# davidsd/sdpb

Hardware: AMD Instinct MI355X
Metric: interior-point iterations/sec at --precision 512 (higher is better)
Workload: dtype mw576 (fixed-width multi-word float, 18x32-bit limbs; Q syrk: exact integer product of a fixed-point image with 509 fraction bits)

## Files before the change

sdpb_amd/csrc/kernels.hpp:

```cpp
#pragma once
#include "dev.hpp"
#include "mw_wave.hpp"
#include "tiledot.hpp"

#include <algorithm>
#include <cmath>
#include <cstdlib>

namespace sdpb
{
using mw::Mw;
using mw::Acc;
constexpr int WG = 256;

template <int NL> MW_HD Mw<NL> mat_ld(const Batch &b, const MatDesc &d, int i, int j)
{
  return mw::load<NL>(b.p, (size_t)d.off + (size_t)i + (size_t)j * (size_t)d.ld);
}
template <int NL> MW_HD void mat_st(const Batch &b, const MatDesc &d, int i, int j, const Mw<NL> &v)
{
  mw::store<NL>(b.p, (size_t)d.off + (size_t)i + (size_t)j * (size_t)d.ld, v);
}

template <int NL, int STRIDE> MW_HD Mw<NL> smem_ld(const uint32_t *s, int idx)
// ... 1794 lines not shown
#endif
}

template <int FX> constexpr bool fx_two_level()
{
#ifdef SDPB_SYRK_ONE_LEVEL
  return false;
#else
  return FX % 4 == 0 && FX <= 32;
#endif
}
template <int NL> constexpr int fx_limbs() { return (NL - 2 >= 14 && (NL - 2) % 4 != 0) ? ((NL - 2 + 3) / 4) * 4 : NL - 2; }
#ifndef SDPB_TOOM4_MAX_FX
#define SDPB_TOOM4_MAX_FX 48
#endif
template <int FX> constexpr bool fx_toom4()
{
#if defined(SDPB_SYRK_ONE_LEVEL) || defined(SDPB_SYRK_NO_TOOM4)
  return false;
#else
  return FX % 4 == 0 && FX >= 16 && FX <= SDPB_TOOM4_MAX_FX;
#endif
}
template <int FX> constexpr bool fx_toom4k()
{
#if defined(SDPB_SYRK_NO_TOOM4K)
  return false;
#else
  return fx_toom4<FX>() && (FX == 16 || FX == 24 || FX == 32);
#endif
}
template <int FX> constexpr bool fx_toom5k()
{
#if defined(SDPB_SYRK_NO_TOOM5K)
  return false;
#else
  return fx_toom4k<FX>() && FX == 16;
#endif
}
constexpr int T5_LB = 28;
constexpr uint32_t T5_MASK = (1u << T5_LB) - 1u;
constexpr int T5_H = 55;
template <int FX> constexpr int fx_nprod() { return fx_toom5k<FX>() ? 27 : 21; }
template <int FX> constexpr int fx_part_limbs() { return fx_toom5k<FX>() ? 5 : 2 * (FX / 8) + 1; }
template <int FX> constexpr int toom_wb() { return fx_toom5k<FX>() ? 102 : 32 * (FX / 4) - (fx_toom4k<FX>() ? 6 : 4); }
template <int FX> constexpr int fx_planes()
{
  return fx_toom5k<FX>() ? 27 * 2 : fx_toom4k<FX>() ? 21 * (FX / 8) : fx_toom4<FX>() ? 7 * (FX / 4) : fx_two_level<FX>() ? 9 * (FX / 4) : 3 * (FX / 2);
}
template <int FX> constexpr int fx_frac_bits()
{
  return fx_toom5k<FX>() ? 5 * toom_wb<FX>() - 1 : fx_toom4<FX>() ? 4 * toom_wb<FX>() - 1 : fx_two_level<FX>() ? 32 * FX - 7 : 32 * FX - 3;
}
template <int FX> constexpr size_t fx_image_stride(size_t rows, size_t cols, int rb)
{
  return fx_toom4k<FX>() ? (rows + rb - 1) / rb * rb * cols + 64 : rows * cols;
}
template <int FX> constexpr int syrk_tile_edge() { return fx_toom4k<FX>() ? 32 : 16; }

template <int BIT0, int NB, int W, int OUT> MW_HD void bits_slice(const uint32_t (&x)[W], uint32_t (&out)[OUT])
{
  constexpr int q = BIT0 / 32, r = BIT0 % 32;
#pragma unroll
  for(int i = 0; i < OUT; ++i)
    {
      const uint32_t lo = (q + i < W) ? x[q + i < W ? q + i : 0] : 0u;
      const uint32_t hi = (q + i + 1 < W) ? x[q + i + 1 < W ? q + i + 1 : 0] : 0u;
      uint32_t v = r ? ((lo >> r) | (hi << ((32 - r) & 31))) : lo;
      const int left = NB - 32 * i;
      if(left <= 0)
        v = 0;
      else if(left < 32)
        v &= (1u << (left & 31)) - 1u;
      out[i] = v;
    }
}

template <int W, int A> MW_HD void add_shifted(uint32_t (&w)[W], const uint32_t (&x)[A], int sh, bool negate)
{
  const int q = sh >> 5, r = sh & 31;
  uint64_t cy = negate ? 1u : 0u;
  const uint32_t mask = negate ? 0xffffffffu : 0u;
#pragma unroll
  for(int k = 0; k < W; ++k)
    {
      const int i0 = k - q;
      uint32_t lo = 0, hi = 0;
#pragma unroll
      for(int t = 0; t < A; ++t)
        {
          lo = (t == i0 - 1) ? x[t] : lo;
          hi = (t == i0) ? x[t] : hi;
        }
      const uint32_t limb = r ? ((hi << r) | (lo >> (32 - r))) : hi;
      const uint64_t s = (uint64_t)w[k] + (uint64_t)(limb ^ mask) + cy;
      w[k] = (uint32_t)s;
      cy = s >> 32;
    }
}

template <int FX> MW_HD void fx_store2(const uint32_t (&mag)[FX], bool negative, uint32_t *fx, size_t fx_stride, size_t idx);
template <int FX> MW_HD void fx_store4(const uint32_t (&mag)[FX], bool negative, uint32_t *fx, size_t fx_stride, size_t idx);
template <int FX> MW_HD void fx_store5(const uint32_t (&mag)[FX], bool negative, uint32_t *fx, size_t fx_stride, size_t idx);
template <int FX> MW_HD void fx_store(const uint32_t (&mag)[FX], bool negative, uint32_t *fx, size_t fx_stride, size_t idx)
{
  constexpr int M = FX / 2;
  static_assert(FX % 2 == 0 && FX >= 4, "FX = NL - 2 is even");
  if constexpr(fx_toom5k<FX>())
    {
// ... 534 lines not shown
    z_sub<Z>(t, w[1]);
#pragma unroll
    for(int k = 0; k < Z; ++k)
      w[1][k] = t[k];
  }
  z_addmul<Z>(w[5], w[3], 8, true);
  z_divexact<Z>(w[5], 9, 0x38E38E39u);
  z_sub<Z>(w[3], w[5]);
  z_divexact<Z>(w[1], 15, 0xEEEEEEEFu);
  z_add<Z>(w[1], w[5]);
  z_sar<Z>(w[1], 1);
  z_sub<Z>(w[5], w[1]);
}

template <int NL, int FX>
__global__ void __launch_bounds__(WG) k_normalize_fx(mw::CPtr PT, size_t count, int N, mw::CPtr inv_norm, uint32_t *fx, size_t fx_stride)
{
  constexpr int FB = fx_frac_bits<FX>();
  for(size_t idx = (size_t)blockIdx.x * WG + threadIdx.x; idx < count; idx += (size_t)gridDim.x * WG)
    {
      const Mw<NL> t = mw::mul(mw::load<NL>(PT, idx), mw::load<NL>(inv_norm, idx % N));
      uint32_t w[NL];
      bool sat = false;
      if(mw::is_zero(t))
        {
#pragma unroll
          for(int i = 0; i < NL; ++i)
            w[i] = 0;
        }
      else
        {
#pragma unroll
          for(int i = 0; i < NL; ++i)
            w[i] = t.m[i];
          const int s = 32 * NL - FB - t.e;
          if(t.e >= 1)
            sat = true;
          else if(s >= 32 * NL)
            {
#pragma unroll
              for(int i = 0; i < NL; ++i)
                w[i] = 0;
            }
          else
            {
              mw::shr_limbs<NL>(w, (uint32_t)s >> 5);
              mw::shr_bits<NL>(w, (uint32_t)s & 31u);
            }
        }
      uint32_t v[FX];
#pragma unroll
      for(int i = 0; i < FX; ++i)
        v[i] = sat ? ((i == FX - 1) ? ((1u << (FB % 32)) - 1u) : 0xffffffffu) : w[i];
      fx_store<FX>(v, t.neg != 0, fx, fx_stride, idx);
    }
}

template <int FX> __global__ void __launch_bounds__(WG) k_fx_from_int(const uint32_t *in, size_t in_stride, size_t count, uint32_t *fx, size_t fx_stride)
{
  const size_t idx = (size_t)blockIdx.x * WG + threadIdx.x;
  if(idx >= count)
    return;
  uint32_t v[FX];
#pragma unroll
  for(int i = 0; i < FX; ++i)
    v[i] = in[(size_t)(i + 1) * in_stride + idx];
  fx_store<FX>(v, in[idx] != 0, fx, fx_stride, idx);
}

template <int FX>
__global__ void __launch_bounds__(WG) k_fx_colsum(const uint32_t *fx, size_t fx_stride, unsigned nrows, int N, unsigned rows_per_slice, uint32_t *partial)
{
  constexpr int M = FX / 2, A = M + 2;
  const int col = blockIdx.x * 64 + (threadIdx.x & 63), phase = threadIdx.x >> 6;
  const unsigned r_begin = blockIdx.y * rows_per_slice, r_end = (r_begin + rows_per_slice < nrows) ? r_begin + rows_per_slice : nrows;
  uint32_t sl[A], sh[A];
#pragma unroll
  for(int k = 0; k < A; ++k)
    sl[k] = sh[k] = 0;
  if(col < N)
    for(unsigned r = r_begin + phase; r < r_end; r += 4)
      {
        const size_t e = (size_t)r * N + col;
        uint64_t cl = 0, ch = 0;
#pragma unroll
        for(int k = 0; k < A; ++k)
          {
            const uint64_t l = (uint64_t)sl[k] + (k < M ? fx[(size_t)(k < M ? k : 0) * fx_stride + e] : 0u) + cl;
            const uint64_t h = (uint64_t)sh[k] + (k < M ? fx[(size_t)(M + (k < M ? k : 0)) * fx_stride + e] : 0u) + ch;
            sl[k] = (uint32_t)l;
            cl = l >> 32;
            sh[k] = (uint32_t)h;
            ch = h >> 32;
          }
      }
  __shared__ uint32_t sm[3 * 2 * A * 64];
  if(phase > 0)
    {
#pragma unroll
      for(int k = 0; k < A; ++k)
        {
          sm[((phase - 1) * 2 * A + k) * 64 + (threadIdx.x & 63)] = sl[k];
          sm[((phase - 1) * 2 * A + A + k) * 64 + (threadIdx.x & 63)] = sh[k];
        }
    }
  __syncthreads();
  if(phase == 0 && col < N)
    {
      for(int p = 0; p < 3; ++p)
        {
          uint64_t cl = 0, ch = 0;
#pragma unroll
          for(int k = 0; k < A; ++k)
            {
              const uint64_t l = (uint64_t)sl[k] + sm[(p * 2 * A + k) * 64 + threadIdx.x] + cl;
              const uint64_t h = (uint64_t)sh[k] + sm[(p * 2 * A + A + k) * 64 + threadIdx.x] + ch;
              sl[k] = (uint32_t)l;
              cl = l >> 32;
              sh[k] = (uint32_t)h;
              ch = h >> 32;
// ... 803 lines not shown
    }
  if constexpr(TOOM)
    {
      if(i < N && j <= i)
        {
          const size_t o = (size_t)tile * 256 + threadIdx.x;
#pragma unroll
          for(int g = 0; g < NG; ++g)
            if(g < ngs)
              {
#pragma unroll
                for(int k = 0; k < A2; ++k)
                  acc[(size_t)((sweep * NG + g) * A2 + k) * acc_stride + o] = g2[g][k];
              }
        }
    }
  else if constexpr(SWEEPS == 3)
    second_level(sweep, 0);
  }
  if constexpr(TOOM)
    return;
  else
  {
  if constexpr(SWEEPS == 1)
    {
#pragma unroll
      for(int k = 0; k < 3; ++k)
        second_level(k, 3 * k);
    }
  if(i < N && j <= i)
    {
      sub_limbs<A>(x[2], x[0]);
      sub_limbs<A>(x[2], x[1]);
      uint32_t w[W];
#pragma unroll
      for(int k = 0; k < W; ++k)
        w[k] = k < A ? x[0][k < A ? k : 0] : 0u;
      add_shifted<W, A>(w, x[2], 32 * M - 3, false);
      add_shifted<W, A>(w, x[1], 64 * M - 6, false);
      const size_t o = packed ? (size_t)tile * 256 + threadIdx.x : (size_t)i + (size_t)j * N;
#pragma unroll
      for(int k = 0; k < W; ++k)
        acc[(size_t)k * acc_stride + o] = w[k];
    }
  }
}

#ifndef SDPB_SYRK3_PREFETCH
#define SDPB_SYRK3_PREFETCH 1
#endif
#ifndef SDPB_SYRK3_WAVES
#define SDPB_SYRK3_WAVES 3
#endif
#ifndef SDPB_SYRK3_NBUF
#define SDPB_SYRK3_NBUF 2
#endif
template <int FX, int RBG>
__global__ void __launch_bounds__(WG, SDPB_SYRK3_WAVES)
  k_syrk_fx3(const uint32_t *__restrict__ fx_in, size_t fx_stride, unsigned nrows, int N, uint32_t *acc, size_t acc_stride,
             const uint32_t *tile_list, int ntile, int nsplit, unsigned rows_per_split, int gsplit, int order)
{
  constexpr bool LAZY = fx_toom5k<FX>();
  constexpr int M3 = FX / 8, A3 = fx_part_limbs<FX>(), NPROD = fx_nprod<FX>();
  static_assert(M3 >= 2 && M3 <= 4 && (!LAZY || (M3 == 2 && RBG <= 32)), "accumulators of 2 x 2 outputs in registers; 2 x 32 rows between carries");
  constexpr int ROWW = 32 * M3, UPR = ROWW / 4, NPAIR = RBG * UPR, GL = NPAIR / WG;
  static_assert(NPAIR % WG == 0, "a pass stages a whole number of units per lane");
  const uint32_t *fx = (const uint32_t *)__builtin_assume_aligned(fx_in, 4);
  const int nitem = ntile * nsplit * gsplit, per = (nitem + 7) / 8;
  int item = (int)(blockIdx.x % 8) * per + (int)(blockIdx.x / 8);
  if(order == 1)
    {
      const int tper = (ntile + 7) / 8, slot = (int)(blockIdx.x / 8), sgx = slot / tper, tl = (int)(blockIdx.x % 8) * tper + slot % tper;
      if(sgx >= nsplit * gsplit || tl >= ntile)
        return;
      item = sgx * ntile + tl;
    }
  else if((int)(blockIdx.x / 8) >= per || item >= nitem)
    return;
  const int sg = item / ntile, tile = item % ntile, split = sg / gsplit;
  const int prod_begin = (sg % gsplit) * (NPROD / gsplit), prod_end = prod_begin + NPROD / gsplit;
  const unsigned row_begin = (unsigned)split * rows_per_split;
  const unsigned row_end = (row_begin + rows_per_split < nrows && split + 1 < nsplit) ? row_begin + rows_per_split : nrows;
  acc += (size_t)split * NPROD * A3 * acc_stride;
  const uint32_t tt = tile_list[tile];
  const int ti = (int)(tt >> 16), tj = (int)(tt & 0xffffu);
  const int li = threadIdx.x & 15, lj = threadIdx.x >> 4;
  const int i0 = ti * 32 + li, j0 = tj * 32 + lj;
  const bool half_i = ti * 32 + 16 < N, half_j = tj * 32 + 16 < N;
  const int mask = 1 | (half_i ? 2 : 0) | ((half_j && tj < ti) ? 4 : 0) | ((half_i && half_j) ? 8 : 0);
#if defined(__HIP_DEVICE_COMPILE__) && !defined(SDPB_SYRK2_NO_GLDS)
  constexpr int NBUF = LAZY ? SDPB_SYRK3_NBUF : 2;
#else
  constexpr int NBUF = 2;
#endif
  static_assert(NBUF == 2 || NBUF == 3, "double or triple buffering");
  __shared__ __attribute__((aligned(16))) uint32_t sa[NBUF * NPAIR * 4 + 64];
  __shared__ __attribute__((aligned(16))) uint32_t sb[NBUF * NPAIR * 4 + 64];
  uint64_t cc[4][2 * M3 - 1];
  uint32_t hh[4][2 * M3 - 1];
  uint64_t dd[4][2 * M3 - 1];
#if defined(__HIP_DEVICE_COMPILE__) && !defined(SDPB_SYRK2_NO_GLDS)
  constexpr bool DIRECT = true;
#else
  constexpr bool DIRECT = false;
#endif
  uint32_t va[DIRECT ? 1 : GL][4], vb[DIRECT ? 1 : GL][4];
  uint32_t offa[GL], offb[GL];
#pragma unroll
  for(int t = 0; t < GL; ++t)
    {
      const int e = threadIdx.x + t * WG;
      const int unit = e % UPR, rr = e / UPR;
      offa[t] = (uint32_t)(((size_t)rr * N + ti * 32) * M3 + 4 * unit);
      offb[t] = (uint32_t)(((size_t)rr * N + tj * 32) * M3 + 4 * unit);
    }
  auto fetch = [&](int g, unsigned r0, int into) __attribute__((always_inline)) {
    const uint32_t *base = fx + ((size_t)g * fx_stride + (size_t)r0 * (size_t)N) * M3;
#pragma unroll
    for(int t = 0; t < GL; ++t)
      {
        if constexpr(DIRECT)
          {
#if defined(__HIP_DEVICE_COMPILE__)
            const int wbase = (into * NPAIR + t * WG + (int)(threadIdx.x & ~63u)) * 4;
            __builtin_amdgcn_global_load_lds((const __attribute__((address_space(1))) void *)(base + offa[t]),
                                             (__attribute__((address_space(3))) void *)(sa + wbase), 16, 0, 0);
            __builtin_amdgcn_global_load_lds((const __attribute__((address_space(1))) void *)(base + offb[t]),
                                             (__attribute__((address_space(3))) void *)(sb + wbase), 16, 0, 0);
#endif
          }
        else
          {
#pragma unroll
            for(int l = 0; l < 4; ++l)
              {
                va[t][l] = base[offa[t] + l];
                vb[t][l] = base[offb[t] + l];
              }
          }
      }
  };
  auto store = [&](int buf) __attribute__((always_inline)) {
    if constexpr(!DIRECT)
      {
#pragma unroll
        for(int t = 0; t < GL; ++t)
          {
            const int e = threadIdx.x + t * WG;
            piece_store<4>(sa + (buf * NPAIR + e) * 4, va[t]);
            piece_store<4>(sb + (buf * NPAIR + e) * 4, vb[t]);
          }
      }
  };
  auto rows = [&](auto mask_c, int buf, uint64_t (&c)[4][2 * M3 - 1], uint32_t (&h)[4][2 * M3 - 1]) __attribute__((always_inline)) {
    constexpr int MASK = decltype(mask_c)::value;
#if defined(__HIP_DEVICE_COMPILE__) && !defined(SDPB_SYRK3_NO_ASM)
    constexpr bool ASM_ROWS = (M3 == 2);
#else
    constexpr bool ASM_ROWS = false;
#endif
    if constexpr(ASM_ROWS)
      {
#if defined(__HIP_DEVICE_COMPILE__)
    typedef uint32_t u32x4 __attribute__((ext_vector_type(4)));
    const uint32_t la = (uint32_t)(uintptr_t)(__attribute__((address_space(3))) uint32_t *)(sa + buf * NPAIR * 4 + li * M3);
    const uint32_t lb = (uint32_t)(uintptr_t)(__attribute__((address_space(3))) uint32_t *)(sb + buf * NPAIR * 4 + lj * M3);
#define FX3_P(C, H, X, Y) "v_mad_u64_u32 %" #C ", vcc, %" #X ", %" #Y ", %" #C "\n\tv_addc_co_u32 %" #H ", vcc, 0, %" #H ", vcc\n\t"
#define FX3_L(C, X, Y) "v_mad_u64_u32 %" #C ", vcc, %" #X ", %" #Y ", %" #C "\n\t"
#define FX3_MAC_BOTH(o0, o1, a0x, a0y, a1x, a1y, bx, by)                                                                                   \
  if constexpr(LAZY)                                                                                                                       \
    asm volatile(FX3_L(0, 6, 10) FX3_L(3, 8, 10) FX3_L(1, 6, 11) FX3_L(4, 8, 11) FX3_L(1, 7, 10) FX3_L(4, 9, 10) FX3_L(2, 7, 11)           \
                   FX3_L(5, 9, 11)                                                                                                         \
                 : "+v"(c[o0][0]), "+v"(c[o0][1]), "+v"(c[o0][2]), "+v"(c[o1][0]), "+v"(c[o1][1]), "+v"(c[o1][2])                          \
                 : "v"(a0x), "v"(a0y), "v"(a1x), "v"(a1y), "v"(bx), "v"(by)                                                                \
                 : "vcc");                                                                                                                 \
  else                                                                                                                                     \
  asm volatile(FX3_P(0, 6, 12, 16) FX3_P(3, 9, 14, 16) FX3_P(1, 7, 12, 17) FX3_P(4, 10, 14, 17) FX3_P(1, 7, 13, 16) FX3_P(4, 10, 15, 16)   \
                 FX3_P(2, 8, 13, 17) FX3_P(5, 11, 15, 17)                                                                                  \
               : "+v"(c[o0][0]), "+v"(c[o0][1]), "+v"(c[o0][2]), "+v"(c[o1][0]), "+v"(c[o1][1]), "+v"(c[o1][2]), "+v"(h[o0][0]),           \
                 "+v"(h[o0][1]), "+v"(h[o0][2]), "+v"(h[o1][0]), "+v"(h[o1][1]), "+v"(h[o1][2])                                            \
               : "v"(a0x), "v"(a0y), "v"(a1x), "v"(a1y), "v"(bx), "v"(by)                                                                  \
               : "vcc")
#define FX3_MAC_ONE(o0, ax, ay, bx, by)                                                                                                    \
  if constexpr(LAZY)                                                                                                                       \
    asm volatile(FX3_L(0, 3, 5) FX3_L(1, 3, 6) FX3_L(1, 4, 5) FX3_L(2, 4, 6)                                                               \
                 : "+v"(c[o0][0]), "+v"(c[o0][1]), "+v"(c[o0][2])                                                                          \
                 : "v"(ax), "v"(ay), "v"(bx), "v"(by)                                                                                      \
                 : "vcc");                                                                                                                 \
  else                                                                                                                                     \
  asm volatile(FX3_P(0, 3, 6, 8) FX3_P(1, 4, 6, 9) FX3_P(1, 4, 7, 8) FX3_P(2, 5, 7, 9)                                                     \
               : "+v"(c[o0][0]), "+v"(c[o0][1]), "+v"(c[o0][2]), "+v"(h[o0][0]), "+v"(h[o0][1]), "+v"(h[o0][2])                            \
               : "v"(ax), "v"(ay), "v"(bx), "v"(by)                                                                                        \
               : "vcc")
#define FX3_ROW(O0, O1)                                                                                                                    \
  {                                                                                                                                        \
    u32x4 va, vb;                    \
    asm volatile("ds_read2_b64 %0, %2 offset0:" #O0 " offset1:" #O1 "\n\tds_read2_b64 %1, %3 offset0:" #O0 " offset1:" #O1                \
                 "\n\ts_waitcnt lgkmcnt(0)"                                                                                                \
                 : "=&v"(va), "=&v"(vb)                                                                                                    \
                 : "v"(xa), "v"(xb)                                                                                                        \
                 : "memory");                                                                                                              \
    if constexpr(MASK == 15)                                                                                                               \
      {                                                                                                                                    \
        FX3_MAC_BOTH(0, 1, va.x, va.y, va.z, va.w, vb.x, vb.y);                                                                            \
        FX3_MAC_BOTH(2, 3, va.x, va.y, va.z, va.w, vb.z, vb.w);                                                                            \
      }                                                                                                                                    \
    else if constexpr(MASK == 11)                                                                                                          \
      {                                                                                                                                    \
        FX3_MAC_BOTH(0, 1, va.x, va.y, va.z, va.w, vb.x, vb.y);                                                                            \
        FX3_MAC_ONE(3, va.z, va.w, vb.z, vb.w);                                                                                            \
      }                                                                                                                                    \
    else if constexpr(MASK == 5)                                                                                                           \
      {                                                                                                                                    \
        FX3_MAC_ONE(0, va.x, va.y, vb.x, vb.y);                                                                                            \
        FX3_MAC_ONE(2, va.x, va.y, vb.z, vb.w);                                                                                            \
      }                                                                                                                                    \
    else                                                                                                                                   \
      FX3_MAC_ONE(0, va.x, va.y, vb.x, vb.y);                                                                                              \
  }
    static_assert(RBG % 4 == 0 && M3 == 2, "four rows per trip, offsets in units of 8 bytes");
#if SDPB_SYRK3_PREFETCH
#define FX3_MACS(va, vb)                                                                                                                   \
  if constexpr(MASK == 15)                                                                                                                 \
    {                                                                                                                                      \
      FX3_MAC_BOTH(0, 1, va.x, va.y, va.z, va.w, vb.x, vb.y);                                                                              \
      FX3_MAC_BOTH(2, 3, va.x, va.y, va.z, va.w, vb.z, vb.w);                                                                              \
    }                                                                                                                                      \
  else if constexpr(MASK == 11)                                                                                                            \
    {                                                                                                                                      \
      FX3_MAC_BOTH(0, 1, va.x, va.y, va.z, va.w, vb.x, vb.y);                                                                              \
      FX3_MAC_ONE(3, va.z, va.w, vb.z, vb.w);                                                                                              \
    }                                                                                                                                      \
  else if constexpr(MASK == 5)                                                                                                             \
    {                                                                                                                                      \
      FX3_MAC_ONE(0, va.x, va.y, vb.x, vb.y);                                                                                              \
      FX3_MAC_ONE(2, va.x, va.y, vb.z, vb.w);                                                                                              \
    }                                                                                                                                      \
  else                                                                                                                                     \
    FX3_MAC_ONE(0, va.x, va.y, vb.x, vb.y);
#ifdef SDPB_SYRK3_EXPERIMENT_HALF_LDS
#define FX3_NEXT(wa, wb, ra, rb, O0, O1)                                                                                                   \
  asm volatile("s_waitcnt lgkmcnt(0)\n\tds_read2_b64 %2, %4 offset0:" #O0 " offset1:" #O1                                                  \
               : "+v"(wa), "+v"(wb), "=&v"(ra), "+v"(rb)                                                                                   \
               : "v"(xa), "v"(xb)                                                                                                          \
               : "memory")
#else
#define FX3_NEXT(wa, wb, ra, rb, O0, O1)                                                                                                   \
  asm volatile("s_waitcnt lgkmcnt(0)\n\tds_read2_b64 %2, %4 offset0:" #O0 " offset1:" #O1 "\n\tds_read2_b64 %3, %5 offset0:" #O0            \
               " offset1:" #O1                                                                                                             \
               : "+v"(wa), "+v"(wb), "=&v"(ra), "=&v"(rb)                                                                                  \
               : "v"(xa), "v"(xb)                                                                                                          \
               : "memory")
#endif
    u32x4 a0, b0, a1, b1;
    {
      const uint32_t xa = la, xb = lb;
      asm volatile("ds_read2_b64 %0, %2 offset0:0 offset1:16\n\tds_read2_b64 %1, %3 offset0:0 offset1:16" : "=&v"(a0), "=&v"(b0) : "v"(xa), "v"(xb) : "memory");
    }
#pragma unroll 1
    for(int rr = 0; rr < RBG; rr += 4)
      {
        const uint32_t xa = la + rr * 256, xb = lb + rr * 256;
        FX3_NEXT(a0, b0, a1, b1, 32, 48);
        FX3_MACS(a0, b0)
        FX3_NEXT(a1, b1, a0, b0, 64, 80);
        FX3_MACS(a1, b1)
        FX3_NEXT(a0, b0, a1, b1, 96, 112);
        FX3_MACS(a0, b0)
        FX3_NEXT(a1, b1, a0, b0, 128, 144);
        FX3_MACS(a1, b1)
      }
    asm volatile("s_waitcnt lgkmcnt(0)" : "+v"(a0), "+v"(b0)::"memory");
#undef FX3_NEXT
#undef FX3_MACS
#else
#pragma unroll 1
    for(int rr = 0; rr < RBG; rr += 4)
      {
        const uint32_t xa = la + rr * 256, xb = lb + rr * 256;
        FX3_ROW(0, 16)
        FX3_ROW(32, 48)
        FX3_ROW(64, 80)
        FX3_ROW(96, 112)
      }
#endif
#undef FX3_ROW
#undef FX3_MAC_ONE
#undef FX3_MAC_BOTH
#undef FX3_P
#undef FX3_L
#endif
      }
    else
      {
        const uint32_t *pa = sa + buf * NPAIR * 4 + li * M3, *pb = sb + buf * NPAIR * 4 + lj * M3;
#pragma unroll SDPB_SYRK2_UNROLL
        for(int rr = 0; rr < RBG; ++rr)
          {
            uint32_t a0[M3], a1[M3], b0[M3], b1[M3];
            piece_load<M3>(pa + rr * ROWW, a0);
            piece_load<M3>(pb + rr * ROWW, b0);
            if constexpr((MASK & 10) != 0)
              piece_load<M3>(pa + rr * ROWW + 16 * M3, a1);
            if constexpr((MASK & 12) != 0)
              piece_load<M3>(pb + rr * ROWW + 16 * M3, b1);
            if constexpr(LAZY)
              {
                auto lazy = [&](const uint32_t (&x)[M3], const uint32_t (&y)[M3], uint64_t (&cs)[2 * M3 - 1]) {
                  cs[0] += (uint64_t)x[0] * y[0];
                  cs[1] += (uint64_t)x[0] * y[1] + (uint64_t)x[1] * y[0];
                  cs[2] += (uint64_t)x[1] * y[1];
                };
                lazy(a0, b0, c[0]);
                if constexpr((MASK & 2) != 0)
                  lazy(a1, b0, c[1]);
                if constexpr((MASK & 4) != 0)
                  lazy(a0, b1, c[2]);
                if constexpr((MASK & 8) != 0)
                  lazy(a1, b1, c[3]);
              }
            else
              {
            SyrkColumns<M3, 0>::run(a0, b0, c[0], h[0]);
            if constexpr((MASK & 2) != 0)
              SyrkColumns<M3, 0>::run(a1, b0, c[1], h[1]);
            if constexpr((MASK & 4) != 0)
              SyrkColumns<M3, 0>::run(a0, b1, c[2], h[2]);
            if constexpr((MASK & 8) != 0)
              SyrkColumns<M3, 0>::run(a1, b1, c[3], h[3]);
              }
          }
      }
  };
  for(int prod = prod_begin; prod < prod_end; ++prod)
    {
#pragma unroll
      for(int o = 0; o < 4; ++o)
#pragma unroll
        for(int k = 0; k < 2 * M3 - 1; ++k)
          {
            cc[o][k] = 0;
            hh[o][k] = 0;
          }
#pragma unroll
      for(int o = 0; o < 4; ++o)
#pragma unroll
        for(int k = 0; k < 2 * M3 - 1; ++k)
          dd[o][k] = 0;
      auto carry_columns = [&](bool all) __attribute__((always_inline)) {
        if constexpr(LAZY)
          {
#pragma unroll
            for(int o = 0; o < 4; ++o)
              {
                dd[o][1] += cc[o][1] >> 32;
                cc[o][1] &= 0xffffffffull;
              }
            if(all)
// ... 103 lines not shown
  const size_t pidx = (size_t)blockIdx.x * WG + threadIdx.x;
  const int prod = blockIdx.y;
  int i, j;
  if(pidx >= total || !syrk_packed_decode<32>(pidx, tile_list, N, col0, col1, i, j))
    return;
  uint32_t out[A3];
  uint64_t cy = 0;
#pragma unroll
  for(int k = 0; k < A3; ++k)
    {
#pragma unroll 8
      for(int s = 0; s < nsplit; ++s)
        cy += part[(((size_t)s * NPROD + prod) * A3 + k) * part_stride + pidx];
      out[k] = (uint32_t)cy;
      cy >>= 32;
    }
#pragma unroll
  for(int k = 0; k < A3; ++k)
    part[((size_t)prod * A3 + k) * part_stride + pidx] = out[k];
}

constexpr uint32_t inv_mod_2_32(uint32_t c)
{
  uint32_t x = c;
  for(int i = 0; i < 5; ++i)
    x *= 2u - c * x;
  return x;
}
constexpr int T5_Z = 10;
MW_HD void toom5_value(const uint32_t *fx, size_t fx_stride, int point, size_t e, uint32_t (&w)[4])
{
  const PiecePair lo = *reinterpret_cast<const PiecePair *>(fx + ((size_t)(3 * point + 0) * fx_stride + e) * 2);
  const PiecePair hi = *reinterpret_cast<const PiecePair *>(fx + ((size_t)(3 * point + 1) * fx_stride + e) * 2);
  w[0] = lo.w[0] | (lo.w[1] << 28);
  w[1] = (lo.w[1] >> 4) | (hi.w[0] << 23);
  w[2] = (hi.w[0] >> 9) | (hi.w[1] << 19);
  w[3] = hi.w[1] >> 13;
}
template <int FX>
__global__ void __launch_bounds__(WG) k_fx_colsum5(const uint32_t *fx, size_t fx_stride, unsigned nrows, int N, unsigned rows_per_slice, uint32_t *partial)
{
  constexpr int A = 5, G = 5;
  const int lane = threadIdx.x & 63, col = blockIdx.x * 64 + lane, phase = threadIdx.x >> 6;
  const unsigned r_begin = blockIdx.y * rows_per_slice, r_end = (r_begin + rows_per_slice < nrows) ? r_begin + rows_per_slice : nrows;
  uint32_t sum[G][A];
#pragma unroll
  for(int u = 0; u < G; ++u)
#pragma unroll
    for(int k = 0; k < A; ++k)
      sum[u][k] = 0;
  if(col < N)
    for(unsigned r = r_begin + phase; r < r_end; r += 4)
      {
        const size_t e = (size_t)r * N + col;
#pragma unroll
        for(int u = 0; u < G; ++u)
          {
            const int point = u == 0 ? 0 : u == 1 ? 1 : u == 2 ? 3 : u == 3 ? 5 : 8;
            uint32_t src[4];
            toom5_value(fx, fx_stride, point, e, src);
            uint64_t cy = 0;
#pragma unroll
            for(int k = 0; k < A; ++k)
              {
                const uint64_t t = (uint64_t)sum[u][k] + (k < 4 ? src[k < 4 ? k : 0] : 0u) + cy;
                sum[u][k] = (uint32_t)t;
                cy = t >> 32;
              }
          }
      }
  __shared__ uint32_t sm[3 * G * A * 64];
  if(phase > 0)
    {
#pragma unroll
      for(int u = 0; u < G; ++u)
#pragma unroll
        for(int k = 0; k < A; ++k)
          sm[(((phase - 1) * G + u) * A + k) * 64 + lane] = sum[u][k];
    }
  __syncthreads();
  if(phase == 0 && col < N)
    {
      for(int p = 0; p < 3; ++p)
#pragma unroll
        for(int u = 0; u < G; ++u)
          {
            uint64_t cy = 0;
#pragma unroll
            for(int k = 0; k < A; ++k)
              {
                const uint64_t t = (uint64_t)sum[u][k] + sm[((p * G + u) * A + k) * 64 + lane] + cy;
                sum[u][k] = (uint32_t)t;
                cy = t >> 32;
              }
          }
#pragma unroll
      for(int u = 0; u < G; ++u)
#pragma unroll
        for(int k = 0; k < A; ++k)
          partial[(((size_t)blockIdx.y * G + u) * A + k) * N + col] = sum[u][k];
    }
}
template <int FX>
__global__ void __launch_bounds__(WG)
  k_fx_colsum5_final(const uint32_t *partial, int nslices, int N, uint32_t *acc, size_t acc_stride, uint32_t *toomU, unsigned long long nrows_local)
{
  constexpr int A = 5, G = 5, W = 2 * FX + 2, WB = toom_wb<FX>(), Z = T5_Z;
// ... 1031 lines not shown
```

sdpb_amd/csrc/solver.hpp:

```cpp
#pragma once
#include "kernels.hpp"
#include "mw_host.hpp"

#include <algorithm>
#include <atomic>
#include <chrono>
#include <cstring>
#include <limits>
#include <map>
#include <memory>
#include <sstream>
#include <string>
#include <utility>

namespace sdpb
{
struct SolverError : std::runtime_error
{
  int code;
  SolverError(int c, const std::string &m) : std::runtime_error(m), code(c) {}
};

struct Collectives
{
// ... 1646 lines not shown
    if(budget_words && need > budget_words)
      {
        const size_t bw = std::max(budget_words, tile_words);
        int nchunk = (int)cdiv(need, bw);
        for(;; ++nchunk)
          {
            int ct = (int)cdiv(ntile, nchunk);
            if(ct >= 64)
              ct = (int)(cdiv(ct, 8) * 8);
            pl.chunk_tiles = std::min(ntile, ct);
            pl.nsplit_first = syrk_splits_for(pl.chunk_tiles, nrows, bw);
            if((size_t)pl.nsplit_first * tile_words * pl.chunk_tiles <= bw || pl.chunk_tiles <= 1)
              break;
          }
        pl.nchunk = (int)cdiv(ntile, pl.chunk_tiles);
      }
    pl.part_words = (size_t)pl.nsplit_first * tile_words * pl.chunk_tiles;
    return pl;
  }
  size_t window_budget_words() const { return max_shared_bytes_ ? std::max<size_t>(1, max_shared_bytes_ / sizeof(uint32_t)) : syrk_part_default_words_; }
  size_t syrk_part_budget_words(size_t image_words) const
  {
    if(const char *e = std::getenv("SDPB_HIP_SYRK_PART_BYTES"))
      return std::max<size_t>(1, (size_t)std::max(1.0, std::atof(e)) / sizeof(uint32_t));
    const size_t w = window_budget_words();
    return std::max<size_t>(1, w - std::min(image_words, w / 2));
  }
  size_t syrk_part_budget_words() const { return syrk_part_budget_words(fx_.n); }
  struct QWindow
  {
    unsigned chunk_rows = 0;
    int chunks = 0;
    size_t stride = 0;
    size_t image_words = 0;
    size_t budget_words = 0;
    bool bound_exceeded = false;
  };
  QWindow qwin_;
  size_t image_budget_words() const
  {
    if(const char *e = std::getenv("SDPB_HIP_SYRK_IMAGE_BYTES"))
      return std::max<size_t>(1, (size_t)std::max(1.0, std::atof(e)) / sizeof(uint32_t));
    return std::max<size_t>(1, window_budget_words() / 2);
  }
  static size_t image_words_for(size_t rows, size_t cols) { return image_stride(rows, cols) * fx_planes<FX>() + 4; }
  QWindow q_window(unsigned nrows, int N, bool one_chunk = false) const
  {
    QWindow w;
    w.budget_words = image_budget_words();
    const unsigned quantum = (unsigned)SYRK_RB;
    unsigned rows = std::max(nrows, 1u);
    if(!one_chunk && image_words_for(rows, (size_t)N) > w.budget_words)
      {
        const size_t per_row = (size_t)N * fx_planes<FX>();
        const size_t fixed = (size_t)64 * fx_planes<FX>() + 4;
        size_t fit = w.budget_words > fixed ? (w.budget_words - fixed) / per_row : 0;
        fit = fit / quantum * quantum;
        if(fit < quantum)
          {
            fit = quantum;
            w.bound_exceeded = true;
          }
        const unsigned f = (unsigned)cdiv(nrows, fit);
        unsigned cr = (unsigned)(cdiv(cdiv(nrows, f), quantum) * quantum);
        if(SYRK_SPLIT_ROWS && cr > SYRK_SPLIT_ROWS)
          {
            const unsigned up = (unsigned)(cdiv(cr, SYRK_SPLIT_ROWS) * SYRK_SPLIT_ROWS);
            if(up <= fit)
              cr = up;
          }
        rows = cr;
      }
    if(one_chunk && image_words_for(rows, (size_t)N) > w.budget_words)
      w.bound_exceeded = true;
    w.chunk_rows = rows;
    w.chunks = nrows ? (int)cdiv(nrows, rows) : 1;
    w.stride = image_stride((size_t)rows, (size_t)N);
    w.image_words = w.stride * fx_planes<FX>() + 4;
    return w;
  }
  template <class MakeImage, class Mark>
  void syrk_G_windows(const QWindow &w, unsigned nrows, int N, DevBuf<uint32_t> &fx, uint32_t *acc, size_t acc_stride, DevBuf<uint32_t> &acc2,
                      uint32_t *colsum_partial, const uint32_t *tiles_dev, DevBuf<uint32_t> &part, uint32_t *toomU, MakeImage &&make, Mark &&mark)
  {
    if(w.chunks > 1 && acc2.n < acc_stride * ACCW)
      acc2.alloc(acc_stride * ACCW);
    for(int c = 0; c < w.chunks; ++c)
      {
        const size_t r0 = (size_t)c * w.chunk_rows;
        const unsigned rows = (unsigned)std::min<size_t>(w.chunk_rows, nrows - r0);
        if(c > 0 && rows < w.chunk_rows)
          HIP_CHECK(hipMemsetAsync(fx.p, 0, fx.n * sizeof(uint32_t), stream_));
        make(r0, rows);
        uint32_t *out = c == 0 ? acc : acc2.p;
        const unsigned slices = (unsigned)std::min<size_t>(128, std::max<size_t>(1, cdiv((size_t)rows, 64)));
        syrk_column_sums(fx.p, w.stride, rows, N, out, acc_stride, colsum_partial, slices, toomU);
        if(c == 0)
          mark();
        syrk_G(fx.p, w.stride, rows, N, out, acc_stride, tiles_dev, part, toomU, -1, 0, -1, w.image_words);
        if(c > 0)
          launch(k_acc_add_tri<ACCW>, dim3(cdiv(acc_stride, WG)), dim3(WG), stream_, acc, (const uint32_t *)acc2.p, acc_stride, N);
      }
    last_windows_ = w.chunks;
  }
  int last_windows_ = 1;
  void syrk_G(const uint32_t *fx, size_t fx_stride, unsigned nrows, int N, uint32_t *acc, size_t acc_stride, const uint32_t *tiles_dev,
              DevBuf<uint32_t> &part, const uint32_t *toomU = nullptr, int ntile_sub = -1, int col0 = 0, int col1 = -1, size_t image_words = 0)
// ... 964 lines not shown
  {
    std::vector<std::pair<const char *, const char *>> tok;
    split_numbers(txt, tok);
    if((int)tok.size() != rows * cols)
      throw SolverError(4, "op_int_syrk: wrong element count");
    const size_t cnt = (size_t)rows * cols;
    std::vector<uint32_t> h(cnt * (FX + 1), 0);
    for(int c = 0; c < cols; ++c)
      for(int r = 0; r < rows; ++r)
        {
          const char *s = tok[(size_t)c * rows + r].first, *e = tok[(size_t)c * rows + r].second;
          bool negative = false;
          if(*s == '-')
            {
              negative = true;
              ++s;
            }
          mw::BigNat n;
          for(; s < e; ++s)
            {
              if(*s < '0' || *s > '9')
                throw SolverError(4, "op_int_syrk: not an integer");
              if(n.w.empty())
                {
                  if(*s != '0')
                    n.w.push_back((uint32_t)(*s - '0'));
                }
              else
                n.mul_small(10, (uint32_t)(*s - '0'));
            }
          if(n.w.size() > (size_t)FX || (n.w.size() == (size_t)FX && (n.w[FX - 1] >> (sdpb::fx_frac_bits<FX>() % 32)) != 0))
            throw SolverError(4, "op_int_syrk: |value| >= 2^" + std::to_string(sdpb::fx_frac_bits<FX>()));
          const size_t idx = (size_t)r * cols + c;
          for(size_t k = 0; k < n.w.size(); ++k)
            h[(k + 1) * cnt + idx] = n.w[k];
          h[idx] = (negative && !n.w.empty()) ? 1u : 0u;
        }
    DevBuf<uint32_t> staged, fx, acc, acc2, partial;
    staged.upload(h);
    const QWindow win = q_window((unsigned)rows, cols);
    image_alloc(fx, win.stride);
    const size_t as = (size_t)cols * cols + cols;
    acc.alloc(as * ACCW);
    const unsigned slices = (unsigned)std::min<size_t>(128, std::max<size_t>(1, cdiv((size_t)rows, 64)));
    partial.alloc((size_t)slices * COLSUM_WORDS * cols);
    DevBuf<uint32_t> tu;
    tu.alloc(TOOMU_WORDS * cols);
    DevBuf<uint32_t> tl;
    tl.upload(syrk_tile_order(cols, 0, nullptr, SYRK_EDGE));
    DevBuf<uint32_t> part;
    syrk_G_windows(win, (unsigned)rows, cols, fx, acc.p, as, acc2, partial.p, (const uint32_t *)tl.p, part, tu.p,
                   [&](size_t r0, unsigned nr) {
                     const size_t n = (size_t)nr * cols;
                     launch(k_fx_from_int<FX>, dim3(cdiv(n, WG)), dim3(WG), stream_, (const uint32_t *)staged.p + r0 * (size_t)cols, cnt, n, fx.p, win.stride);
                   },
                   [] {});
    launch(k_syrk_unbias<FX>, dim3(cdiv((size_t)cols * cols, WG)), dim3(WG), stream_, acc.p, as, cols, (unsigned long long)rows, (size_t)0,
           (size_t)cols * cols);
    HIP_CHECK(hipStreamSynchronize(stream_));
    std::vector<uint32_t> a = acc.download();
    std::string out;
    for(int j = 0; j < cols; ++j)
      for(int i = 0; i < cols; ++i)
        {
          const size_t idx = (size_t)i + (size_t)j * cols;
          if(i < j)
            {
              out += "0\n";
              continue;
            }
          mw::BigNat n;
          n.w.resize(ACCW);
          for(int k = 0; k < ACCW; ++k)
            n.w[k] = a[(size_t)k * as + idx];
          const bool negative = n.w[ACCW - 1] >> 31;
          if(negative)
            {
              uint64_t carry = 1;
              for(auto &w : n.w)
                {
                  const uint64_t s = (uint64_t)(~w) + carry;
                  w = (uint32_t)s;
                  carry = s >> 32;
                }
            }
          n.trim();
          std::string dig;
          while(!n.is_zero())
            {
              uint32_t rem = n.div_small(1000000000u);
              for(int k = 0; k < 9; ++k)
                {
                  dig.push_back((char)('0' + rem % 10));
                  rem /= 10;
                }
            }
          while(!dig.empty() && dig.back() == '0')
            dig.pop_back();
          if(dig.empty())
            dig = "0";
          else if(negative)
            dig.push_back('-');
          out.append(dig.rbegin(), dig.rend());
          out += "\n";
        }
    return out;
  }
// ... 14 lines not shown
```

sdpb_amd/workmodel.py:

```python
from __future__ import annotations

from typing import Dict, Sequence


def shapes(dims: Sequence[int], num_points: Sequence[int]):
    for m, K in zip(dims, num_points):
        P = K * m * (m + 1) // 2
        n0 = m * ((K + 1) // 2)
        n1 = m * K - n0
        yield m, K, P, (n0, n1), m * K


def macs_per_iteration(dims, num_points, N) -> Dict[str, float]:
    w = dict(cholesky_XY=0.0, pairings=0.0, schur=0.0, schur_cholesky=0.0, schur_trsm=0.0, syrk_Q=0.0,
             cholesky_Q=0.0, XY=0.0, search_direction=0.0, step_length=0.0, residues=0.0)
    for m, K, P, ns, q in shapes(dims, num_points):
        for n in ns:
            w["cholesky_XY"] += 2 * n ** 3 / 3.0
            w["pairings"] += 2.5 * n * n * q + n * q * q
            w["XY"] += n ** 3
            w["search_direction"] += 2 * 7 * n ** 3
            w["step_length"] += 2 * (2 * n ** 3 + 6 * n ** 3)
            w["residues"] += n * n * K
        w["schur"] += 8.0 * P * P
# ... 16 lines not shown
        t += 4 * q * q + P * P
        t += P * P + 2 * P * N
        t += P * N
    t += N * (N + 1) / 2 + N * N
    return t * bytes_per_number


COMPILED_LIMBS = (6, 10, 16, 18, 24, 26, 34, 42, 50, 66)
HBM_BYTES = 288 * 10 ** 9


def limbs_for(precision: int) -> int:
    want = 2 * ((precision + 127) // 64)
    for nl in COMPILED_LIMBS:
        if nl >= want:
            return nl
    raise ValueError(f"--precision {precision} is beyond the compiled widths")


def _fx(nl: int):
    fx = nl - 2
    if fx >= 14 and fx % 4:
        fx += 4 - fx % 4
    toom4 = fx >= 16 and fx % 4 == 0
    toom4k = fx in (16, 24, 32)
    toom5k = fx == 16
    two = fx % 4 == 0
    words = 54 if toom5k else 21 * (fx // 8) if toom4k else 7 * (fx // 4) if toom4 else 9 * (fx // 4) if two else 3 * (fx // 2)
    planes = 135 if toom5k else 21 * (2 * (fx // 8) + 1) if toom4k else 7 * (2 * (fx // 4) + 1) if toom4 else 2 * fx + 2
    rb = (16 if fx >= 32 else 32) if two else (16 if fx <= 24 else 8)
    waves = 3 if toom4k else (3 if fx <= 16 else 2)
    return fx, words, 32 if toom4k else 16, planes, rb, waves, toom4, toom4k


def syrk_row_splits(ntile: int, nrows: int, slots: int, rb: int, max_rows: int) -> int:
    import math
    smin = 1
    while max_rows and smin < 32 and nrows // smin > max_rows and nrows // (smin + 1) >= 64 * rb:
        smin += 1
    best, best_eff = smin, 0.0
    for s in range(smin, 33):
        if s > smin and nrows // s < 64 * rb:
            break
        items = ntile * s
        eff = items / (math.ceil(items / slots) * slots)
        if eff > best_eff + 0.02:
            best, best_eff = s, eff
    return best


def q_window(rows: int, N: int, nl: int, image_budget_bytes: int):
    fx, words, edge, planes, rb, waves, toom4, toom4k = _fx(nl)

    def image_bytes(r):
        stride = (-(-r // rb) * rb * N + 64) if toom4k else r * N
        return (max(stride, 1) * words + 4) * 4
    r = max(rows, 1)
    budget_words = max(1, image_budget_bytes // 4)
    if image_bytes(r) // 4 > budget_words:
        per_row = N * words
        fixed = 64 * words + 4
        fit = ((budget_words - fixed) // per_row if budget_words > fixed else 0) // rb * rb
        fit = max(fit, rb)
        f = -(-rows // fit)
        cr = -(-(-(-rows // f)) // rb) * rb
        if toom4k and cr > 2560:
            up = -(-cr // 2560) * 2560
            if up <= fit:
                cr = up
        r = cr
    return r, (-(-rows // r) if rows else 1), image_bytes(r)


def planned_footprint(dims, num_points, N, precision, owners=None, rank=0, world=1, num_cus=256, hbm_bytes=HBM_BYTES,
                      max_shared_bytes=0, dist_cholq=False, free_bytes=None) -> Dict[str, float]:
    nl = limbs_for(precision)
    W = 4 * (nl + 1)
    fx, words, edge, planes, rb, waves, toom4, toom4k = _fx(nl)
    psd = bases = scaled = E = pair = schur = bt = vecn = rows = jl = 0
    for j, (m, K, P, ns, q) in enumerate(shapes(dims, num_points)):
        if owners is not None and owners[j] != rank:
            continue
        jl += 1
        d = K - 1
        pr = m * (m + 1) // 2
        for n, r in zip(ns, (d // 2 + 1, (d + 1) // 2)):
            psd += n * n
            vecn += n
            bases += r * K
            scaled += K * pr * r
            E += n * q
            pair += q * q
        schur += P * P
        bt += N * P
        rows += P
    out = {"psd_state_and_scratch": 13 * max(psd, 1) * W, "bases_and_pairings": (2 * max(bases, 1) + max(scaled, 1) + 4 * max(E, 1) + 2 * max(pair, 1)) * W,
           "schur_blocks": 2 * max(schur, 1) * W, "B": max(bt, 1) * W, "P": max(bt, 1) * W}
    accw = 2 * fx + 2
    q_bytes = 2 * N * N * W + (N * N + N) * accw * 4
    if world > 1:
        q_bytes += (N * (N + 1) // 2 + N) * accw * 8
        if dist_cholq:
            pb = 16 if nl > 34 else 32
            q_bytes += ((N * pb + pb * pb + pb) * (nl + 1) + 2) * 4
    out["Q"] = q_bytes
    out["vectors_and_small"] = (5 * max(rows, 1) + 6 * max(vecn, 1) + 8 * N + 2 * max(jl, 1) * N) * W
    rest = sum(out.values())
    free = (hbm_bytes if free_bytes is None else free_bytes) - rest
    reserve = hbm_bytes // 16 + (1 << 30)
    window = max_shared_bytes or max(min(max(free - reserve, 0), hbm_bytes // 8), 64 << 20)
    chunk_rows, windows, image = q_window(rows, N, nl, max(window // 2, 4))
    out["P_fixed_point_image"] = image
    if windows > 1:
# ... 19 lines not shown
```

Measured before the change: 6.141.

## Interleave column slots in toom5k fixed-point image for 128-bit LDS reads

Changes the fixed-point image layout for the toom5k path so that columns c and c+16 within each 32-column group sit in adjacent slots, with rows padded to a multiple of 32. The lazy syrk inner loop can then fetch both operands for a row with a single ds_read_b128 instead of ds_read2_b64, and it is unrolled over 8, 16 or 32-row trips. Producers, the colsum kernel, window sizing and the Python work model are updated to the new addressing. This adds padding memory and index arithmetic on the image writers, and depends on every consumer agreeing on the permutation.

```diff
diff --git a/sdpb_amd/csrc/kernels.hpp b/sdpb_amd/csrc/kernels.hpp
--- a/sdpb_amd/csrc/kernels.hpp
+++ b/sdpb_amd/csrc/kernels.hpp
@@ -1870,9 +1870,18 @@
 {
   return fx_toom5k<FX>() ? 5 * toom_wb<FX>() - 1 : fx_toom4<FX>() ? 4 * toom_wb<FX>() - 1 : fx_two_level<FX>() ? 32 * FX - 7 : 32 * FX - 3;
 }
+template <int FX> constexpr int fx_col_slot(int c) { return fx_toom5k<FX>() ? 32 * (c / 32) + 2 * (c % 16) + (c % 32) / 16 : c; }
+template <int FX> constexpr size_t fx_row_slots(size_t cols) { return fx_toom5k<FX>() ? (cols + 31) / 32 * 32 : cols; }
+template <int FX> MW_HD size_t fx_elem(size_t idx, int N)
+{
+  if constexpr(fx_toom5k<FX>())
+    return idx / (size_t)N * fx_row_slots<FX>((size_t)N) + (size_t)fx_col_slot<FX>((int)(idx % (size_t)N));
+  else
+    return idx;
+}
 template <int FX> constexpr size_t fx_image_stride(size_t rows, size_t cols, int rb)
 {
-  return fx_toom4k<FX>() ? (rows + rb - 1) / rb * rb * cols + 64 : rows * cols;
+  return fx_toom4k<FX>() ? (rows + rb - 1) / rb * rb * fx_row_slots<FX>(cols) + 64 : rows * cols;
 }
 template <int FX> constexpr int syrk_tile_edge() { return fx_toom4k<FX>() ? 32 : 16; }
 
@@ -2513,11 +2522,12 @@
 #pragma unroll
       for(int i = 0; i < FX; ++i)
         v[i] = sat ? ((i == FX - 1) ? ((1u << (FB % 32)) - 1u) : 0xffffffffu) : w[i];
-      fx_store<FX>(v, t.neg != 0, fx, fx_stride, idx);
-    }
-}
-
-template <int FX> __global__ void __launch_bounds__(WG) k_fx_from_int(const uint32_t *in, size_t in_stride, size_t count, uint32_t *fx, size_t fx_stride)
+      fx_store<FX>(v, t.neg != 0, fx, fx_stride, fx_elem<FX>(idx, N));
+    }
+}
+
+template <int FX>
+__global__ void __launch_bounds__(WG) k_fx_from_int(const uint32_t *in, size_t in_stride, size_t count, int N, uint32_t *fx, size_t fx_stride)
 {
   const size_t idx = (size_t)blockIdx.x * WG + threadIdx.x;
   if(idx >= count)
@@ -2526,7 +2536,7 @@
 #pragma unroll
   for(int i = 0; i < FX; ++i)
     v[i] = in[(size_t)(i + 1) * in_stride + idx];
-  fx_store<FX>(v, in[idx] != 0, fx, fx_stride, idx);
+  fx_store<FX>(v, in[idx] != 0, fx, fx_stride, fx_elem<FX>(idx, N));
 }
 
 template <int FX>
@@ -3436,6 +3446,9 @@
 #ifndef SDPB_SYRK3_WAVES
 #define SDPB_SYRK3_WAVES 3
 #endif
+#ifndef SDPB_SYRK3_LAZY_TRIP
+#define SDPB_SYRK3_LAZY_TRIP 32
+#endif
 #ifndef SDPB_SYRK3_NBUF
 #define SDPB_SYRK3_NBUF 2
 #endif
@@ -3488,6 +3501,7 @@
 #else
   constexpr bool DIRECT = false;
 #endif
+  const size_t NS = fx_row_slots<FX>((size_t)N);
   uint32_t va[DIRECT ? 1 : GL][4], vb[DIRECT ? 1 : GL][4];
   uint32_t offa[GL], offb[GL];
 #pragma unroll
@@ -3495,11 +3509,11 @@
     {
       const int e = threadIdx.x + t * WG;
       const int unit = e % UPR, rr = e / UPR;
-      offa[t] = (uint32_t)(((size_t)rr * N + ti * 32) * M3 + 4 * unit);
-      offb[t] = (uint32_t)(((size_t)rr * N + tj * 32) * M3 + 4 * unit);
+      offa[t] = (uint32_t)(((size_t)rr * NS + ti * 32) * M3 + 4 * unit);
+      offb[t] = (uint32_t)(((size_t)rr * NS + tj * 32) * M3 + 4 * unit);
     }
   auto fetch = [&](int g, unsigned r0, int into) __attribute__((always_inline)) {
-    const uint32_t *base = fx + ((size_t)g * fx_stride + (size_t)r0 * (size_t)N) * M3;
+    const uint32_t *base = fx + ((size_t)g * fx_stride + (size_t)r0 * NS) * M3;
 #pragma unroll
     for(int t = 0; t < GL; ++t)
       {
@@ -3547,8 +3561,9 @@
       {
 #if defined(__HIP_DEVICE_COMPILE__)
     typedef uint32_t u32x4 __attribute__((ext_vector_type(4)));
-    const uint32_t la = (uint32_t)(uintptr_t)(__attribute__((address_space(3))) uint32_t *)(sa + buf * NPAIR * 4 + li * M3);
-    const uint32_t lb = (uint32_t)(uintptr_t)(__attribute__((address_space(3))) uint32_t *)(sb + buf * NPAIR * 4 + lj * M3);
+    constexpr int LSTEP = LAZY ? 2 * M3 : M3;
+    const uint32_t la = (uint32_t)(uintptr_t)(__attribute__((address_space(3))) uint32_t *)(sa + buf * NPAIR * 4 + li * LSTEP);
+    const uint32_t lb = (uint32_t)(uintptr_t)(__attribute__((address_space(3))) uint32_t *)(sb + buf * NPAIR * 4 + lj * LSTEP);
 #define FX3_P(C, H, X, Y) "v_mad_u64_u32 %" #C ", vcc, %" #X ", %" #Y ", %" #C "\n\tv_addc_co_u32 %" #H ", vcc, 0, %" #H ", vcc\n\t"
 #define FX3_L(C, X, Y) "v_mad_u64_u32 %" #C ", vcc, %" #X ", %" #Y ", %" #C "\n\t"
 #define FX3_MAC_BOTH(o0, o1, a0x, a0y, a1x, a1y, bx, by)                                                                                   \
@@ -3602,8 +3617,16 @@
     else                                                                                                                                   \
       FX3_MAC_ONE(0, va.x, va.y, vb.x, vb.y);                                                                                              \
   }
+#define FX3L_ROW(ROW)                                                                                                                      \
+  {                                                                                                                                        \
+    u32x4 va, vb;                                                                                                                          \
+    asm volatile("ds_read_b128 %0, %2 offset:%4\n\tds_read_b128 %1, %3 offset:%4\n\ts_waitcnt lgkmcnt(0)"                                  \
+                 : "=&v"(va), "=&v"(vb)                                                                                                    \
+                 : "v"(xa), "v"(xb), "n"((ROW) * 256)                                                                                      \
+                 : "memory");                                                                                                              \
+    FX3_MACS(va, vb)                                                                                                                       \
+  }
     static_assert(RBG % 4 == 0 && M3 == 2, "four rows per trip, offsets in units of 8 bytes");
-#if SDPB_SYRK3_PREFETCH
 #define FX3_MACS(va, vb)                                                                                                                   \
   if constexpr(MASK == 15)                                                                                                                 \
     {                                                                                                                                      \
@@ -3622,6 +3645,7 @@
     }                                                                                                                                      \
   else                                                                                                                                     \
     FX3_MAC_ONE(0, va.x, va.y, vb.x, vb.y);
+#if SDPB_SYRK3_PREFETCH
 #ifdef SDPB_SYRK3_EXPERIMENT_HALF_LDS
 #define FX3_NEXT(wa, wb, ra, rb, O0, O1)                                                                                                   \
   asm volatile("s_waitcnt lgkmcnt(0)\n\tds_read2_b64 %2, %4 offset0:" #O0 " offset1:" #O1                                                  \
@@ -3636,38 +3660,95 @@
                : "v"(xa), "v"(xb)                                                                                                          \
                : "memory")
 #endif
+#define FX3L_NEXT(wa, wb, ra, rb, ROW)                                                                                                     \
+  asm volatile("s_waitcnt lgkmcnt(0)\n\tds_read_b128 %2, %4 offset:%6\n\tds_read_b128 %3, %5 offset:%6"                                   \
+               : "+v"(wa), "+v"(wb), "=&v"(ra), "=&v"(rb)                                                                                  \
+               : "v"(xa), "v"(xb), "n"((ROW) * 256)                                                                                        \
+               : "memory")
+#define FX3L_ROWS2(R)                                                                                                                      \
+  FX3L_NEXT(a0, b0, a1, b1, (R) + 1);                                                                                                      \
+  FX3_MACS(a0, b0)                                                                                                                         \
+  FX3L_NEXT(a1, b1, a0, b0, (R) + 2);                                                                                                      \
+  FX3_MACS(a1, b1)
+#define FX3L_ROWS8(R) FX3L_ROWS2(R) FX3L_ROWS2((R) + 2) FX3L_ROWS2((R) + 4) FX3L_ROWS2((R) + 6)
     u32x4 a0, b0, a1, b1;
-    {
-      const uint32_t xa = la, xb = lb;
-      asm volatile("ds_read2_b64 %0, %2 offset0:0 offset1:16\n\tds_read2_b64 %1, %3 offset0:0 offset1:16" : "=&v"(a0), "=&v"(b0) : "v"(xa), "v"(xb) : "memory");
-    }
+    if constexpr(LAZY)
+      {
+        constexpr int TRIP = (RBG % SDPB_SYRK3_LAZY_TRIP == 0) ? SDPB_SYRK3_LAZY_TRIP : 8;
+        static_assert(RBG % 8 == 0 && (TRIP == 8 || TRIP == 16 || TRIP == 32) && RBG * 256 < 65536, "whole trips, the offsets fit 16 bits");
+        {
+          const uint32_t xa = la, xb = lb;
+          asm volatile("ds_read_b128 %0, %2\n\tds_read_b128 %1, %3" : "=&v"(a0), "=&v"(b0) : "v"(xa), "v"(xb) : "memory");
+        }
 #pragma unroll 1
-    for(int rr = 0; rr < RBG; rr += 4)
+        for(int rr = 0; rr < RBG; rr += TRIP)
+          {
+            const uint32_t xa = la + rr * 256, xb = lb + rr * 256;
+            FX3L_ROWS8(0)
+            if constexpr(TRIP >= 16)
+              {
+                FX3L_ROWS8(8)
+              }
+            if constexpr(TRIP >= 32)
+              {
+                FX3L_ROWS8(16)
+                FX3L_ROWS8(24)
+              }
+          }
+      }
+    else
       {
-        const uint32_t xa = la + rr * 256, xb = lb + rr * 256;
-        FX3_NEXT(a0, b0, a1, b1, 32, 48);
-        FX3_MACS(a0, b0)
-        FX3_NEXT(a1, b1, a0, b0, 64, 80);
-        FX3_MACS(a1, b1)
-        FX3_NEXT(a0, b0, a1, b1, 96, 112);
-        FX3_MACS(a0, b0)
-        FX3_NEXT(a1, b1, a0, b0, 128, 144);
-        FX3_MACS(a1, b1)
+        {
+          const uint32_t xa = la, xb = lb;
+          asm volatile("ds_read2_b64 %0, %2 offset0:0 offset1:16\n\tds_read2_b64 %1, %3 offset0:0 offset1:16" : "=&v"(a0), "=&v"(b0) : "v"(xa), "v"(xb) : "memory");
+        }
+#pragma unroll 1
+        for(int rr = 0; rr < RBG; rr += 4)
+          {
+            const uint32_t xa = la + rr * 256, xb = lb + rr * 256;
+            FX3_NEXT(a0, b0, a1, b1, 32, 48);
+            FX3_MACS(a0, b0)
+            FX3_NEXT(a1, b1, a0, b0, 64, 80);
+            FX3_MACS(a1, b1)
+            FX3_NEXT(a0, b0, a1, b1, 96, 112);
+            FX3_MACS(a0, b0)
+            FX3_NEXT(a1, b1, a0, b0, 128, 144);
+            FX3_MACS(a1, b1)
+          }
       }
     asm volatile("s_waitcnt lgkmcnt(0)" : "+v"(a0), "+v"(b0)::"memory");
+#undef FX3L_ROWS8
+#undef FX3L_ROWS2
+#undef FX3L_NEXT
 #undef FX3_NEXT
+#else
+    if constexpr(LAZY)
+      {
+#pragma unroll 1
+        for(int rr = 0; rr < RBG; rr += 4)
+          {
+            const uint32_t xa = la + rr * 256, xb = lb + rr * 256;
+            FX3L_ROW(0)
+            FX3L_ROW(1)
+            FX3L_ROW(2)
+            FX3L_ROW(3)
+          }
+      }
+    else
+      {
+#pragma unroll 1
+        for(int rr = 0; rr < RBG; rr += 4)
+          {
+            const uint32_t xa = la + rr * 256, xb = lb + rr * 256;
+            FX3_ROW(0, 16)
+            FX3_ROW(32, 48)
+            FX3_ROW(64, 80)
+            FX3_ROW(96, 112)
+          }
+      }
+#endif
 #undef FX3_MACS
-#else
-#pragma unroll 1
-    for(int rr = 0; rr < RBG; rr += 4)
-      {
-        const uint32_t xa = la + rr * 256, xb = lb + rr * 256;
-        FX3_ROW(0, 16)
-        FX3_ROW(32, 48)
-        FX3_ROW(64, 80)
-        FX3_ROW(96, 112)
-      }
-#endif
+#undef FX3L_ROW
 #undef FX3_ROW
 #undef FX3_MAC_ONE
 #undef FX3_MAC_BOTH
@@ -3677,7 +3758,8 @@
       }
     else
       {
-        const uint32_t *pa = sa + buf * NPAIR * 4 + li * M3, *pb = sb + buf * NPAIR * 4 + lj * M3;
+        constexpr int LSTEP = LAZY ? 2 * M3 : M3, SECOND = LAZY ? M3 : 16 * M3;
+        const uint32_t *pa = sa + buf * NPAIR * 4 + li * LSTEP, *pb = sb + buf * NPAIR * 4 + lj * LSTEP;
 #pragma unroll SDPB_SYRK2_UNROLL
         for(int rr = 0; rr < RBG; ++rr)
           {
@@ -3685,9 +3767,9 @@
             piece_load<M3>(pa + rr * ROWW, a0);
             piece_load<M3>(pb + rr * ROWW, b0);
             if constexpr((MASK & 10) != 0)
-              piece_load<M3>(pa + rr * ROWW + 16 * M3, a1);
+              piece_load<M3>(pa + rr * ROWW + SECOND, a1);
             if constexpr((MASK & 12) != 0)
-              piece_load<M3>(pb + rr * ROWW + 16 * M3, b1);
+              piece_load<M3>(pb + rr * ROWW + SECOND, b1);
             if constexpr(LAZY)
               {
                 auto lazy = [&](const uint32_t (&x)[M3], const uint32_t (&y)[M3], uint64_t (&cs)[2 * M3 - 1]) {
@@ -3897,7 +3979,7 @@
   if(col < N)
     for(unsigned r = r_begin + phase; r < r_end; r += 4)
       {
-        const size_t e = (size_t)r * N + col;
+        const size_t e = (size_t)r * fx_row_slots<FX>((size_t)N) + (size_t)fx_col_slot<FX>(col);
 #pragma unroll
         for(int u = 0; u < G; ++u)
           {
diff --git a/sdpb_amd/csrc/solver.hpp b/sdpb_amd/csrc/solver.hpp
--- a/sdpb_amd/csrc/solver.hpp
+++ b/sdpb_amd/csrc/solver.hpp
@@ -1722,7 +1722,7 @@
     unsigned rows = std::max(nrows, 1u);
     if(!one_chunk && image_words_for(rows, (size_t)N) > w.budget_words)
       {
-        const size_t per_row = (size_t)N * fx_planes<FX>();
+        const size_t per_row = fx_row_slots<FX>((size_t)N) * fx_planes<FX>();
         const size_t fixed = (size_t)64 * fx_planes<FX>() + 4;
         size_t fit = w.budget_words > fixed ? (w.budget_words - fixed) / per_row : 0;
         fit = fit / quantum * quantum;
@@ -2793,7 +2793,8 @@
     syrk_G_windows(win, (unsigned)rows, cols, fx, acc.p, as, acc2, partial.p, (const uint32_t *)tl.p, part, tu.p,
                    [&](size_t r0, unsigned nr) {
                      const size_t n = (size_t)nr * cols;
-                     launch(k_fx_from_int<FX>, dim3(cdiv(n, WG)), dim3(WG), stream_, (const uint32_t *)staged.p + r0 * (size_t)cols, cnt, n, fx.p, win.stride);
+                     launch(k_fx_from_int<FX>, dim3(cdiv(n, WG)), dim3(WG), stream_, (const uint32_t *)staged.p + r0 * (size_t)cols, cnt, n, cols,
+                            fx.p, win.stride);
                    },
                    [] {});
     launch(k_syrk_unbias<FX>, dim3(cdiv((size_t)cols * cols, WG)), dim3(WG), stream_, acc.p, as, cols, (unsigned long long)rows, (size_t)0,
diff --git a/sdpb_amd/workmodel.py b/sdpb_amd/workmodel.py
--- a/sdpb_amd/workmodel.py
+++ b/sdpb_amd/workmodel.py
@@ -92,13 +92,15 @@
 def q_window(rows: int, N: int, nl: int, image_budget_bytes: int):
     fx, words, edge, planes, rb, waves, toom4, toom4k = _fx(nl)
 
+    slots = -(-N // 32) * 32 if fx == 16 else N
+
     def image_bytes(r):
-        stride = (-(-r // rb) * rb * N + 64) if toom4k else r * N
+        stride = (-(-r // rb) * rb * slots + 64) if toom4k else r * N
         return (max(stride, 1) * words + 4) * 4
     r = max(rows, 1)
     budget_words = max(1, image_budget_bytes // 4)
     if image_bytes(r) // 4 > budget_words:
-        per_row = N * words
+        per_row = slots * words
         fixed = 64 * words + 4
         fit = ((budget_words - fixed) // per_row if budget_words > fixed else 0) // rb * rb
         fit = max(fit, rb)
```

Result: faster. 6.284 (median of 6 runs) (+2.3%).
